# Graph-Machine-Learning-Group/sgp

Measured on AMD Instinct MI355X. Metric: encoded node-steps/sec, higher is better.
Workload: dtype f32 (hop products: operands as fp16 hi + lo pairs, three 16-bit MFMA terms per product, fp32 accumulation -- agrees with fp32 to ~1e-7 of the operand scale; reservoir: recurrent products: state (|h| <= 1, x 2^14) and W_hh (per-row power-of-two scale) as two fp16 pieces (22 bits), hi*hi + hi*lo + lo*

## Files before the change

include/sgp_amd.h:

```cpp
#ifndef SGP_AMD_H
#define SGP_AMD_H

#include <stdint.h>

#ifdef __cplusplus
extern "C" {
#endif

#define SGP_ABI_VERSION 4

#define SGP_EINVAL   (-1)
#define SGP_EUNSUP   (-2)
#define SGP_ENOMEM   (-3)

#define SGP_ACT_TANH      0
#define SGP_ACT_RELU      1
#define SGP_ACT_SELF_NORM 2
#define SGP_ACT_IDENTITY  3
#define SGP_ACT_TANH_REL  4

typedef void* sgp_stream_t;

int sgp_abi_version(void);
const char* sgp_last_error(void);
// ... 68 lines not shown
                       const float* x_tab, int32_t accumulate, int32_t t_chunk, const int32_t* pred, int32_t run_if, sgp_stream_t stream);
int32_t sgp_spmm_split_chunks(void);
int32_t sgp_spmm_split_max_union(void);
int32_t sgp_spmm_split_waves(void);
int32_t sgp_spmm_split_rows_per_wave(void);
int32_t sgp_spmm_split_max_feat(void);

int sgp_spmm_split_banded_f32(const int32_t* hdr, const int32_t* rowid, const int32_t* ucol, const void* afr,
                              const int32_t* adr, const float* rinv, int32_t n_tiles,
                              const float* X, int64_t x_row_stride, int64_t x_batch_stride,
                              const float* X_halo, int64_t xh_row_stride, int64_t xh_batch_stride, int32_t n_own,
                              float* Y, int64_t y_row_stride, int64_t y_batch_stride,
                              int32_t n_rows, int32_t n_cols, int32_t batch, int32_t feat,
                              const float* x_tab, int32_t accumulate, int32_t t_chunk,
                              int32_t walk, const int32_t* band_first, int32_t n_bands,
                              const int32_t* pred, int32_t run_if, sgp_stream_t stream);

int sgp_spmm_split_wide_f32(const int32_t* hdr, const int32_t* rowid, const int32_t* ucol, const void* afr,
                            const int32_t* adr, const float* rinv, int32_t n_tiles,
                            const float* X, int64_t x_row_stride, int64_t x_batch_stride,
                            const float* X_halo, int64_t xh_row_stride, int64_t xh_batch_stride, int32_t n_own,
                            float* Y, int64_t y_row_stride, int64_t y_batch_stride,
                            int32_t n_rows, int32_t n_cols, int32_t batch, int32_t feat,
                            const float* x_tab, int32_t accumulate, int32_t t_chunk, const int32_t* pred, int32_t run_if, sgp_stream_t stream);
int sgp_spmm_split_wide_banded_f32(const int32_t* hdr, const int32_t* rowid, const int32_t* ucol, const void* afr,
                                   const int32_t* adr, const float* rinv, int32_t n_tiles,
                                   const float* X, int64_t x_row_stride, int64_t x_batch_stride,
                                   const float* X_halo, int64_t xh_row_stride, int64_t xh_batch_stride, int32_t n_own,
                                   float* Y, int64_t y_row_stride, int64_t y_batch_stride,
                                   int32_t n_rows, int32_t n_cols, int32_t batch, int32_t feat,
                                   const float* x_tab, int32_t accumulate, int32_t t_chunk,
                                   int32_t walk, const int32_t* band_first, int32_t n_bands,
                                   const int32_t* pred, int32_t run_if, sgp_stream_t stream);
int32_t sgp_spmm_split_wide_chunks(void);
int32_t sgp_spmm_split_wide_max_union(void);
int32_t sgp_spmm_split_wide_waves(void);
int32_t sgp_spmm_split_wide_rows_per_wave(void);
int32_t sgp_spmm_split_wide_max_feat(void);

int sgp_split_plan_order(const int64_t* rowptr, const int64_t* col, int64_t nnz, int64_t n_rows, int64_t n_cols,
                         int32_t waves, int32_t chunks, int32_t max_union, int32_t rows_per_wave, int64_t* order);
int64_t sgp_split_plan_deal(const int64_t* rowptr, const int64_t* col, int64_t nnz, int64_t n_rows, int64_t n_cols,
                            const int64_t* order, int64_t n_order,
                            int32_t waves, int32_t chunks, int32_t max_union, int32_t rows_per_wave,
                            int64_t* wave_of_row, int64_t* slot_of_row, int64_t* tile_of_wave, int64_t* rows_of_wave);
int sgp_split_plan_fill(const int64_t* rowptr, const int64_t* col, const float* val, int64_t nnz, int64_t n_rows, int64_t n_cols,
                        const int64_t* wave_of_row, const int64_t* slot_of_row, const int64_t* tile_of_wave,
                        const int64_t* rows_of_wave, int64_t n_waves, int64_t n_tiles,
                        int32_t waves, int32_t chunks, int32_t max_union,
                        int32_t* hdr, int32_t* rowid, int32_t* ucol, void* afr, int32_t* adr, float* rinv,
                        double* stats, int32_t threads);
int64_t sgp_split_plan_bands(const int32_t* ucol, int64_t n_tiles, int32_t max_union, int64_t n_cols,
                             int64_t col_budget, int32_t* band_first);

int sgp_spmm_colblock_f32(const int32_t* plan, const int32_t* segptr, const int32_t* wg_row0,
                          int32_t n_wg, int32_t n_blocks,
                          const float* X, int64_t x_row_stride, int64_t x_batch_stride,
                          const float* X_halo, int64_t xh_row_stride, int64_t xh_batch_stride, int32_t n_own,
                          float* Y, int64_t y_row_stride, int64_t y_batch_stride,
                          int32_t n_rows, int32_t n_cols, int32_t batch, int32_t feat,
                          const int32_t* pred, int32_t run_if, sgp_stream_t stream);
int32_t sgp_spmm_colblock_rows_cap(void);
int32_t sgp_spmm_colblock_round_pad(void);

int32_t sgp_spmm_tiled_max_union(int32_t feat);
int32_t sgp_spmm_tiled_max_tile_rows(void);
int32_t sgp_spmm_tiled_max_row_edges(void);

int sgp_spmm_tiled_form(int32_t tile_rows, int32_t max_row_edges, int32_t* rows_per_group, int32_t* batches);
int32_t sgp_spmm_csr_form(int32_t feat, int32_t aligned, int32_t predicated);

int64_t sgp_reservoir_workspace_bytes(int32_t F, int32_t R);
int sgp_reservoir_f32(const float* x, int64_t x_row_stride, int64_t x_step_stride,
                      const float* w_ih, const float* w_hh, const float* b,
                      double alpha, int32_t act,
                      float* out, int64_t out_row_stride, int64_t out_step_stride,
                      float* h_state, void* workspace,
                      int32_t T, int32_t N, int32_t F, int32_t R,
                      sgp_stream_t stream);

int sgp_reservoir_pieces_f32(const float* x, int64_t x_row_stride, int64_t x_step_stride,
                             const float* w_ih, const float* w_hh, const float* b,
                             double alpha, int32_t act,
                             float* out, int64_t out_row_stride, int64_t out_step_stride,
                             float* h_state, void* workspace,
                             int32_t t_piece, int32_t t_last, int32_t n_pieces,
                             int64_t x_piece_stride, int64_t out_piece_stride, int32_t no_store,
                             int32_t N, int32_t F, int32_t R,
                             const int32_t* pred, int32_t run_if, sgp_stream_t stream);

int sgp_reservoir_describe(int32_t F, int32_t R, int32_t N, int32_t T, int32_t act, double alpha, int32_t has_state,
                           int32_t n_pieces, int32_t no_store, int32_t has_pred,
                           int64_t x_row_stride, int64_t x_step_stride, int32_t x_align,
                           int64_t out_row_stride, int64_t out_step_stride, int32_t out_align,
                           char* text, int64_t capacity);

int64_t sgp_reservoir_fused_workspace_bytes(int32_t F, int32_t R, int32_t L);
int32_t sgp_reservoir_fused_supported(int32_t F, int32_t R, int32_t L);
int sgp_reservoir_fused_f32(const float* x, int64_t x_row_stride, int64_t x_step_stride,
                            const float* const* w_ih, const float* const* w_hh, const float* const* b,
                            const double* alpha, int32_t act,
                            float* out, int64_t out_row_stride, int64_t out_step_stride,
                            float* h_state, void* workspace,
                            int32_t T, int32_t N, int32_t F, int32_t R, int32_t L,
                            sgp_stream_t stream);
int sgp_reservoir_fused_sums_f32(const float* x, int64_t x_row_stride, int64_t x_step_stride,
// ... 397 lines not shown
```

sgp_amd/csrc/plan_split.hip:

```cpp
#include "common.h"
#include <math.h>
#include <string.h>
#include <algorithm>
#include <atomic>
#include <new>
#include <system_error>
#include <thread>
#include <vector>

namespace {

constexpr int SET_SLOTS[4][8] = {{0, 1, 2, 3, 8, 9, 10, 11}, {4, 5, 6, 7, 12, 13, 14, 15},
                                 {16, 17, 18, 19, 24, 25, 26, 27}, {20, 21, 22, 23, 28, 29, 30, 31}};

inline uint16_t half_bits(_Float16 h) { uint16_t b; memcpy(&b, &h, 2); return b; }

inline void split_fp16(float v, uint16_t& hi, uint16_t& lo) {
    uint32_t bits;
    memcpy(&bits, &v, 4);
    bits &= 0xFFFFE000u;
    float hi32;
    memcpy(&hi32, &bits, 4);
    if (fabsf(v) < 6.103515625e-05f) hi32 = (float)(_Float16)v;
    const _Float16 h = (_Float16)hi32;
// ... 327 lines not shown
            w_mark[c] = wave;
            ++w_union;
            for (int64_t i = g.cp[c]; i < g.cp[c + 1]; ++i) {
                const int32_t q = g.cr[i];
                if (in_tile[q] != tile) continue;
                if (w_cnt_at[q] != wave) { w_cnt_at[q] = wave; w_cnt[q] = 0; }
                ++w_cnt[q];
            }
        }
    }
    int32_t cut_waves() {
        rest.assign(rows.begin(), rows.end());
        std::sort(rest.begin(), rest.end());
        for (int32_t r : rest) in_tile[r] = tile;
        wave_rows.clear();
        wave_first.assign(1, 0);
        while (!rest.empty()) {
            ++wave;
            w_union = 0;
            int32_t n_in = 0;
            size_t at = 0;
            for (;;) {
                const int32_t r = rest[at];
                rest.erase(rest.begin() + (int64_t)at);
                wave_take(r);
                if (++n_in == rows_per_wave || rest.empty()) break;
                at = 0;
                for (size_t i = 1; i < rest.size(); ++i) {
                    const int32_t q = rest[i], b = rest[at];
                    const int32_t nq = g.deg(q) - w_have(q), nb = g.deg(b) - w_have(b);
                    if (nq < nb || (nq == nb && w_have(q) > w_have(b))) at = i;
                }
                if (w_union + g.deg(rest[at]) - w_have(rest[at]) > wave_cols) break;
            }
            wave_first.push_back((int32_t)wave_rows.size());
        }
        return (int32_t)wave_first.size() - 1;
    }
    void run(int64_t* order) {
        int64_t n_out = 0;
        while (n_out < n_rows) {
            grow_tile();
            const int32_t n_waves = cut_waves();
            const int32_t kept = std::min(n_waves, waves);
            for (int32_t i = 0; i < wave_first[kept]; ++i) order[n_out++] = wave_rows[i];
            for (int32_t i = wave_first[kept]; i < wave_first[n_waves]; ++i) {
                placed[wave_rows[i]] = 0;
                next_row = std::min<int64_t>(next_row, wave_rows[i]);
            }
        }
    }
};

}

extern "C" int sgp_split_plan_order(const int64_t* rowptr, const int64_t* col, int64_t nnz, int64_t n_rows, int64_t n_cols,
                                    int32_t waves, int32_t chunks, int32_t max_union, int32_t rows_per_wave, int64_t* order) {
  return guarded<int>("sgp_split_plan_order", [&]() -> int {
    SGP_REQUIRE(rowptr && (col || nnz <= 0) && order, "sgp_split_plan_order: null pointer");
    SGP_REQUIRE(n_rows >= 0 && n_cols >= 0 && n_rows < (1ll << 31) - 1 && n_cols < (1ll << 31) - 1 && waves >= 1 && chunks >= 1 &&
                chunks <= (1 << 24) && max_union >= 1 && rows_per_wave >= 1 && (int64_t)waves * rows_per_wave < (1ll << 31),
                "sgp_split_plan_order: bad size");
    if (const char* f = rowptr_fault(rowptr, n_rows, nnz)) return sgp::fail(SGP_EINVAL, "sgp_split_plan_order: malformed CSR: %s", f);
    if (n_rows == 0) return 0;
    OrderGraph g;
    if (const char* f = order_graph(rowptr, col, n_rows, n_cols, g)) return sgp::fail(SGP_EINVAL, "sgp_split_plan_order: %s", f);
    Orderer(g, n_rows, n_cols, waves, chunks, max_union, rows_per_wave).run(order);
    return 0;
  });
}

extern "C" int sgp_split_plan_fill(const int64_t* rowptr, const int64_t* col, const float* val, int64_t nnz, int64_t n_rows, int64_t n_cols,
                                   const int64_t* wave_of_row, const int64_t* slot_of_row, const int64_t* tile_of_wave,
                                   const int64_t* rows_of_wave, int64_t n_waves, int64_t n_tiles,
                                   int32_t waves, int32_t chunks, int32_t max_union,
                                   int32_t* hdr, int32_t* rowid, int32_t* ucol, void* afr, int32_t* adr, float* rinv,
                                   double* stats, int32_t threads) {
  return guarded<int>("sgp_split_plan_fill", [&]() -> int {
    SGP_REQUIRE(rowptr && col && val && wave_of_row && slot_of_row && tile_of_wave && rows_of_wave && hdr && rowid && ucol &&
                afr && adr && rinv && stats, "sgp_split_plan_fill: null pointer");
    SGP_REQUIRE(n_rows > 0 && n_cols > 0 && n_waves > 0 && n_tiles > 0 && waves >= 1 && 2 * waves < 64 && chunks >= 1 &&
                max_union >= 1 && max_union <= 65536 / 64 * 8, "sgp_split_plan_fill: bad size");
    if (const char* f = rowptr_fault(rowptr, n_rows, nnz)) return sgp::fail(SGP_EINVAL, "sgp_split_plan_fill: malformed CSR: %s", f);
    for (int64_t e = 0; e < rowptr[n_rows]; ++e)
        SGP_REQUIRE(col[e] >= 0 && col[e] < n_cols, "sgp_split_plan_fill: column out of range");
    FillArgs a{rowptr, col, val, n_rows, n_cols, wave_of_row, slot_of_row, tile_of_wave, rows_of_wave, n_waves, n_tiles,
               waves, chunks, max_union, hdr, rowid, ucol, (uint16_t*)afr, adr, rinv};
    memset(hdr, 0, sizeof(int32_t) * 64 * n_tiles);
    std::fill(rowid, rowid + n_tiles * waves * 16, -1);
    std::fill(ucol, ucol + n_tiles * (int64_t)max_union, -1);
    memset(afr, 0, sizeof(uint16_t) * (size_t)n_tiles * waves * chunks * 2 * 512);
    memset(adr, 0, sizeof(int32_t) * (size_t)n_tiles * waves * chunks * 64);
    memset(rinv, 0, sizeof(float) * (size_t)n_tiles * waves * 16);
    std::vector<int64_t> first_wave(n_tiles + 1, 0), row_first(n_waves + 1, 0);
    for (int64_t w = 0; w < n_waves; ++w) {
        const int64_t t = tile_of_wave[w];
        SGP_REQUIRE(t >= 0 && t < n_tiles && (w == 0 || t == tile_of_wave[w - 1] || t == tile_of_wave[w - 1] + 1),
                    "sgp_split_plan_fill: tile_of_wave is not a non-decreasing run");
        SGP_REQUIRE(rows_of_wave[w] >= 0 && rows_of_wave[w] <= 16, "sgp_split_plan_fill: a wave holds at most 16 rows");
        ++first_wave[t + 1];
        row_first[w + 1] = row_first[w] + rows_of_wave[w];
    }
    for (int64_t t = 0; t < n_tiles; ++t) {
        SGP_REQUIRE(first_wave[t + 1] >= 1 && first_wave[t + 1] <= waves, "sgp_split_plan_fill: a tile holds 1 .. waves waves");
        first_wave[t + 1] += first_wave[t];
    }
// ... 90 lines not shown
```

sgp_amd/graph.py:

```python
from typing import NamedTuple

import numpy as np
import torch

from . import hip, tune
from .tileplan import build_reordered_plan, build_tile_plan, locality_order


def _as_edge_tensors(edge_index, edge_weight):
    if isinstance(edge_index, np.ndarray):
        edge_index = torch.from_numpy(edge_index)
        if edge_weight is not None and isinstance(edge_weight, np.ndarray):
            edge_weight = torch.from_numpy(edge_weight)
    if not torch.is_tensor(edge_index):
        raise RuntimeError("Edge index must be (edge_index, edge_weight) tuple "
                           "or SparseTensor.")
    ei = edge_index.detach().to("cpu", torch.long)
    ew = None if edge_weight is None else edge_weight.detach().to("cpu", torch.float32)
    return ei, ew


def _coalesce(row, col, val, n):
    key = row * n + col
    uniq, inv = torch.unique(key, sorted=True, return_inverse=True)
# ... 218 lines not shown
        key = ("colblock", feat, str(device))
        if key not in self._plans:
            plan = None
            from . import colblock
            if feat % 64 == 0 and self.num_cols < colblock.MAX_COLS and self.nnz() > 0:
                lib = hip.load()
                plan = colblock.build_colblock_plan(self.rowptr.numpy(), self.col.numpy(), self.val.numpy(),
                                                    self.num_nodes, self.num_cols, feat,
                                                    rows_cap=lib.sgp_spmm_colblock_rows_cap(),
                                                    round_pad=lib.sgp_spmm_colblock_round_pad(),
                                                    l2_bytes=tune.get("colblock_l2_mb", 2.5, float) * 2 ** 20)
                if plan is not None:
                    plan = plan.to(device)
            self._plans[key] = plan
        return self._plans[key]

    def mix_plan(self, feat, device, strict=True):
        key = ("mix", feat % 64 == 0, str(device), bool(strict))
        if key not in self._plans:
            plan = None
            base = self.tile_plan(feat, device, tall=False)
            if base is not None and base.pipe is not None and (base.group_fill >= 0.5 or not strict):
                from . import mixplan, plancache
                lib = hip.load()
                thr, dh = tune.get("mix_thr", 4, int), lib.sgp_spmm_mix_max_dense(int(self.num_cols > self.num_nodes))

                def build():
                    order = None
                    if base.reordered:
                        order = locality_order(self.rowptr.numpy(), self.col.numpy(), self.num_nodes)
                    return mixplan.build_mix_plan(self.rowptr.numpy(), self.col.numpy(), self.val.numpy(), self.num_nodes,
                                                  base, thr=thr, dh=dh, order=order)
                plan = plancache.fetch(self, "mix", (thr, dh, sorted(hip.tiled_limits(feat).items())), build)
                min_share = tune.get("mix_min_share", 0.25, float) if strict else -1.0
                if plan is not None and (plan.dense_share < min_share
                                         or plan.max_union > lib.sgp_spmm_mix_max_union()):
                    plan = None
                if plan is not None:
                    plan = plan.to(device)
            self._plans[key] = plan
        return self._plans[key]

    def split_plan(self, device):
        key = ("split", str(device))
        if key not in self._plans:
            plan = None
            if self.nnz() > 0:
                from . import plancache
                lib = hip.load()
                lim, wide = hip.split_limits(), hip.split_limits(wide=True)
                if tune.get("split_wide", 1, int) == 0:
                    wide = None
                plan = plancache.fetch(self, "split", (sorted(lim.items()), wide and sorted(wide.items()),
                                                       tune.get("split_passes", 1, int), _split_order_mode()),
                                       lambda: self._build_split_plan(lim, wide))
                if isinstance(plan, list):
                    plan = SplitPasses(p.to(device) for p in plan)
                elif plan is not None:
                    plan = plan.to(device)
            self._plans[key] = plan
        return self._plans[key]

    def _build_split_plan(self, lim, wide=None):
        from . import splitplan
        args = (self.rowptr.numpy(), self.col.numpy(), self.val.numpy(), self.num_nodes, self.num_cols)
        bands = dict(band_cols=SPLIT_BAND_BYTES // 256)
        plan = splitplan.build_split_plan(*args, **lim, **bands)
        if plan is not None and plan.stats["rows_per_wave"] < 0.75 * lim["rows_per_wave"] and self.num_nodes >= 2048 and \
                self.num_cols == self.num_nodes:
            alt = splitplan.build_split_plan(*args, order=locality_order(
                self.rowptr.numpy(), self.col.numpy(), self.num_nodes), **lim, **bands)
            if alt is not None and alt.stats["staged_per_row"] < plan.stats["staged_per_row"]:
                plan = alt
                plan.stats["order"] = "locality"
        mode = _split_order_mode()
        if plan is not None and mode != "off" and self.num_cols == self.num_nodes:
            given = plan.stats["tiles"]
            blob = splitplan.blob_order(*args[:2], *args[3:], **lim)
            tiles = splitplan.deal_tiles(*args[:2], *args[3:], order=blob, **lim)
            if tiles is not None and (tiles < given or mode == "on"):
                plan = splitplan.build_split_plan(*args, order=blob, **lim, **bands)
                plan.stats["order"] = "blob"
            plan.stats.setdefault("order", "numbering")
            plan.stats.update(split_order=mode, tiles_given=given, tiles_blob=tiles)
        if plan is not None and (plan.stats["rows_per_wave"] < 0.375 * lim["rows_per_wave"] or
                                 plan.stats["staged_per_row"] > 8):
            plan = None
        if plan is None and self.max_degree() > 32 * lim["chunks"] and tune.get("split_passes", 1, int) != 0:
            deg = (self.rowptr[1:] - self.rowptr[:-1])
            if wide is not None and float((deg > 32 * lim["chunks"]).float().mean()) < 0.5:
                wide = None
            passes = splitplan.build_split_passes(*args, max_passes=12, **(wide or lim), **bands)
            if passes is not None and passes[0].stats["rows_per_wave"] >= 0.5 * lim["rows_per_wave"] and \
                    passes[0].stats["staged_per_row"] <= 8:
                plan = list(passes)
            elif wide is not None:
                return self._build_split_plan(lim, None)
        return plan

    def prepare(self, feat, device, halo=False):
        self.device_csr(device)
        if self.nnz() == 0:
            return ["csr"]
        c = self._select(feat, device, _NOMINAL)
        made = (["split"] if c.split is not None else []) + (["tile"] if c.tile is not None else [])
        if c.lazy:
            return made + ["csr (behind the split hop's predicate until a flag asks for the exact kernels)"]
        made += {"spmm_mix": ["mix"], "spmm_colblock": ["colblock"]}.get(c.kernel, [])
        return made or ["csr"]

    def split_eligible(self, x, y, halo=None):
        return self._select(x.shape[2], x.device, _operands(x, y, halo, None), split_only=True).split is not None

    def norm_inf(self):
        if not hasattr(self, "_norm_inf"):
            rp = self.rowptr.long()
            sums = torch.zeros(self.num_nodes, dtype=torch.float64)
            if self.nnz():
                sums.index_add_(0, torch.repeat_interleave(torch.arange(self.num_nodes), rp[1:] - rp[:-1]),
                                self.val.double().abs())
            self._norm_inf = float(sums.max()) if self.num_nodes else 0.0
        return self._norm_inf

    def propagate(self, x, y, force=None, halo=None, x_bound=None):
        if (halo is None) != (self.num_cols == self.num_nodes):
            raise ValueError("halo rows are required exactly when num_cols > num_nodes")
        if x.dim() != 3 or y.dim() != 3 or y.shape[0] != x.shape[0] or y.shape[2] != x.shape[2]:
            raise ValueError("propagate expects [B, N, F] operands of equal batch and feature size")
        n_src = x.shape[1] + (0 if halo is None else halo.shape[1])
        if n_src != self.num_cols or y.shape[1] != self.num_nodes:
            raise ValueError(f"operand shapes do not match the operator: {n_src} source rows for "
                             f"{self.num_cols} columns, {y.shape[1]} result rows for {self.num_nodes}")
        if halo is not None and (halo.shape[0] != x.shape[0] or halo.shape[2] != x.shape[2]):
            raise ValueError("halo batch / feature size differs from x")
        if force not in (None, "csr", "tiled", "res", "mix", "colblock", "split"):
            raise ValueError(f"unknown kernel {force!r} (csr, tiled, res, mix, colblock, split)")
        if x.shape[0] == 0 or x.shape[2] == 0 or self.num_nodes == 0:
# ... 118 lines not shown
        if not self._flag_pending:
            return
        still = []
        for slot, ev in self._flag_pending:
            if ev.query():
                if int(self._flag_host[slot]) == 0:
                    self._exact_seen = True
            else:
                still.append((slot, ev))
        self._flag_pending = still

    def index_select(self, dim, index):
        if dim != 0:
            raise NotImplementedError("only row selection (dim=0) is used by the reference")
        idx = torch.as_tensor(index, dtype=torch.long).cpu()
        rp = self.rowptr.long()
        counts = (rp[1:] - rp[:-1])[idx]
        new_rp = torch.zeros(idx.numel() + 1, dtype=torch.long)
        new_rp[1:] = torch.cumsum(counts, 0)
        take = torch.repeat_interleave(rp[idx] - new_rp[:-1], counts) + torch.arange(int(new_rp[-1]))
        return ShiftOperator(new_rp, self.col[take], self.val[take], idx.numel(), num_cols=self.num_cols)

    def propagate_rect(self, x, y):
        if x.shape[1] != self.num_cols or y.shape[1] != self.num_nodes:
            raise ValueError("operand shapes do not match the operator")
        if self.num_cols == self.num_nodes:
            return self.propagate(x, y)
        rowptr, col, val = self.device_csr(x.device)
        hip.spmm_csr(rowptr, col, val, x, y)
        return y

    def __matmul__(self, x):
        if not torch.is_tensor(x) or x.dim() < 2:
            raise TypeError("ShiftOperator @ expects a dense tensor [..., N, F]")
        lead = x.shape[:-2]
        x3 = x.reshape(-1, x.shape[-2], x.shape[-1])
        if x3.dtype != torch.float32:
            x3 = x3.float()
        if x3.stride(2) != 1:
            x3 = x3.contiguous()
        if x3.shape[1] != self.num_cols:
            raise ValueError(f"operand has {x3.shape[1]} rows, the operator {self.num_cols} columns")
        on_cpu = not x3.is_cuda
        if on_cpu:
            hip.require_gpu()
            x3 = x3.cuda()
        y = torch.empty(x3.shape[0], self.num_nodes, x3.shape[2], dtype=torch.float32, device=x3.device)
        self.propagate_rect(x3, y)
        if on_cpu:
            y = y.cpu()
        return y.reshape(*lead, self.num_nodes, x.shape[-1])


def _split_order_mode():
    mode = tune.get("split_order", "auto")
    if mode not in ("off", "on", "auto"):
        raise ValueError(f"SGP_TUNE: split_order={mode!r} is not one of off, on, auto")
    return mode


class SplitPasses(list):

    @property
    def stats(self):
        return self[0].stats

    @property
    def n_tiles(self):
        return sum(p.n_tiles for p in self)
```

sgp_amd/plancache.py:

```python
import hashlib
import os
import tempfile

import torch

VERSION = 9
_dir = None
stats = {"hits": 0, "misses": 0, "stores": 0}


def set_dir(path):
    global _dir
    _dir = path


def directory():
    return _dir or os.environ.get("SGP_AMD_CACHE") or None


def operator_hash(op):
    h = getattr(op, "_csr_hash", None)
    if h is None:
        m = hashlib.blake2b(digest_size=16)
        m.update(f"{op.num_nodes}:{op.num_cols}:{op.nnz()}".encode())
        for t in (op.rowptr, op.col, op.val):
            m.update(t.contiguous().numpy().tobytes())
        h = op._csr_hash = m.hexdigest()
    return h


def _path(op, kind, params):
    d = directory()
    if d is None:
        return None
    tag = hashlib.blake2b(repr((VERSION, kind, params)).encode(), digest_size=8).hexdigest()
    return os.path.join(d, f"{kind}-{operator_hash(op)}-{tag}.pt")


_MISS = object()


def fetch(op, kind, params, build):
    path = _path(op, kind, params)
    if path is None:
        return build()
    if os.path.exists(path):
        try:
            got = torch.load(path, map_location="cpu", weights_only=False)
            if isinstance(got, dict) and got.get("version") == VERSION and got.get("params") == repr(params):
                stats["hits"] += 1
                return got["plan"]
        except Exception:
            pass
    stats["misses"] += 1
    plan = build()
    try:
        os.makedirs(os.path.dirname(path), exist_ok=True)
        fd, tmp = tempfile.mkstemp(dir=os.path.dirname(path), suffix=".tmp")
        os.close(fd)
# ... 7 lines not shown
```

sgp_amd/splitplan.py:

```python
import numpy as np
import torch


class SplitPlan:
    def __init__(self, hdr, rowid, ucol, afr, adr, rinv, n_tiles, n_rows, n_cols, norm_inf, stats):
        self.hdr, self.rowid, self.ucol, self.afr, self.adr, self.rinv = hdr, rowid, ucol, afr, adr, rinv
        self.n_tiles, self.n_rows, self.n_cols = n_tiles, n_rows, n_cols
        self.norm_inf, self.stats = norm_inf, stats
        self.accumulate = False
        self.bands = {}
        self.ucol_host = ucol if ucol.device.type == "cpu" else None

    def __setstate__(self, state):
        self.__dict__.update(state)
        self.__dict__.setdefault("bands", {})
        self.__dict__.setdefault("ucol_host", self.ucol if self.ucol.device.type == "cpu" else None)

    def to(self, device):
        p = SplitPlan(self.hdr.to(device), self.rowid.to(device), self.ucol.to(device), self.afr.to(device),
                      self.adr.to(device), self.rinv.to(device), self.n_tiles, self.n_rows, self.n_cols, self.norm_inf,
                      self.stats)
        p.accumulate = self.accumulate
        p.bands = {k: (t.to(device), m) for k, (t, m) in self.bands.items()}
        p.ucol_host = self.ucol_host
        return p

    def band_table(self, col_budget):
        col_budget = int(col_budget)
        if col_budget not in self.bands:
            host = self.ucol_host if self.ucol_host is not None else self.ucol.cpu()
            first = build_bands(host, self.n_cols, col_budget)
            self.bands[col_budget] = (first.to(self.ucol.device), int((first[1:] - first[:-1]).max()))
        return self.bands[col_budget]

    def describe(self):
        st = self.stats
        line = (f"split plan: {st['tiles']} tiles, {st['rows_per_tile']:.1f} rows per tile, {st['rows_per_wave']:.2f} rows per wave, "
                f"{st['staged_per_row']:.2f} staged rows per result row")
        if "order" in st:
            line += (f"; rows dealt in {st['order']} order (SGP_TUNE split_order={st['split_order']}: "
                     f"{st['tiles_given']} tiles in the given order, {st['tiles_blob']} in blob order)")
        return line


def build_bands(ucol, n_cols, col_budget):
    from . import hip
    lib = hip.load()
    ucol = ucol.contiguous()
    assert ucol.dtype == torch.int32 and ucol.dim() == 2 and ucol.device.type == "cpu"
    n_tiles = ucol.shape[0]
    first = torch.empty(n_tiles + 1, dtype=torch.int32)
    n = lib.sgp_split_plan_bands(ucol.data_ptr(), n_tiles, ucol.shape[1], int(n_cols), int(col_budget), first.data_ptr())
    if n < 0:
        raise (MemoryError if n == -3 else RuntimeError)("sgp_split_plan_bands: " + lib.sgp_last_error().decode())
    return first[:n + 1].clone()


def _host_csr(rowptr, col, n_rows):
    rowptr = np.ascontiguousarray(rowptr, dtype=np.int64)
    col = np.ascontiguousarray(col, dtype=np.int64)
    if rowptr.size < n_rows + 1:
        raise ValueError("rowptr is shorter than n_rows + 1")
    return rowptr, col


def blob_order(rowptr, col, n_rows, n_cols, waves=16, chunks=7, max_union=768, rows_per_wave=16):
    import ctypes
    from . import hip
    lib = hip.load()
    rowptr, col = _host_csr(rowptr, col, n_rows)
    ptr = lambda a: a.ctypes.data_as(ctypes.c_void_p)
    order = np.empty(n_rows, dtype=np.int64)
    rc = lib.sgp_split_plan_order(ptr(rowptr), ptr(col), col.size, n_rows, n_cols, waves, chunks, max_union, rows_per_wave, ptr(order))
    if rc != 0:
        raise (MemoryError if rc == -3 else ValueError)("sgp_split_plan_order: " + lib.sgp_last_error().decode())
    return order


def deal_tiles(rowptr, col, n_rows, n_cols, waves=16, chunks=7, max_union=768, rows_per_wave=16, order=None):
    import ctypes
    from . import hip
    lib = hip.load()
    rowptr, col = _host_csr(rowptr, col, n_rows)
    seq = None if order is None else np.ascontiguousarray(order, dtype=np.int64)
    ptr = lambda a: a.ctypes.data_as(ctypes.c_void_p)
    out = [np.empty(max(n_rows, 1), dtype=np.int64) for _ in range(4)]
    n_waves = lib.sgp_split_plan_deal(ptr(rowptr), ptr(col), col.size, n_rows, n_cols, None if seq is None else ptr(seq),
                                      0 if seq is None else seq.size, waves, chunks, max_union, rows_per_wave, *map(ptr, out))
    if n_waves == -2 or n_waves == 0:
        return None
    if n_waves < 0:
        raise (MemoryError if n_waves == -3 else RuntimeError)("sgp_split_plan_deal: " + lib.sgp_last_error().decode())
    return int(out[2][n_waves - 1]) + 1


def deal_rows(rowptr, col, n_rows, n_cols, waves, chunks, max_union, rows_per_wave=32, order=None):
    cap = 32 * chunks
    wmark = np.full(n_cols, -1, dtype=np.int64)
    tmark = np.full(n_cols, -1, dtype=np.int64)
    wave_of_row = np.full(n_rows, -1, dtype=np.int64)
    slot_of_row = np.full(n_rows, -1, dtype=np.int64)
    tile_of_wave, rows = [], []
    wave, tile = -1, -1
    w_rows = w_cols = t_cols = t_waves = 0

    def open_wave(r, new_tile):
        nonlocal wave, tile, w_rows, w_cols, t_cols, t_waves
        wave += 1
        if new_tile:
            tile += 1
            t_cols = t_waves = 0
        t_waves += 1
        w_rows = w_cols = 0
        tile_of_wave.append(tile)
        rows.append(0)

    for r in (range(n_rows) if order is None else order):
        r = int(r)
        c = np.unique(col[rowptr[r]:rowptr[r + 1]])
        if c.size > cap or c.size > max_union:
            return None
        if wave < 0:
            open_wave(r, True)
        new_w = int((wmark[c] != wave).sum())
        new_t = int((tmark[c] != tile).sum())
        need_wave = w_rows == rows_per_wave or w_cols + new_w > cap
        if t_cols + new_t > max_union or (need_wave and t_waves == waves):
            open_wave(r, True)
            new_w = new_t = c.size
        elif need_wave:
            open_wave(r, False)
            new_w = c.size
        wmark[c] = wave
        tmark[c] = tile
        w_cols += new_w
        t_cols += new_t
        wave_of_row[r] = wave
        slot_of_row[r] = w_rows
        w_rows += 1
        rows[wave] = w_rows
    return (wave_of_row, slot_of_row, np.asarray(tile_of_wave, dtype=np.int64), np.asarray(rows, dtype=np.int64))


def split_fp16(v):
    v = np.asarray(v, dtype=np.float32)
    bits = v.view(np.uint32) & np.uint32(0xFFFFE000)
    hi32 = bits.view(np.float32)
    small = np.abs(v) < np.float32(2.0 ** -14)
    hi32 = np.where(small, v.astype(np.float16).astype(np.float32), hi32)
    hi = hi32.astype(np.float16)
    lo = (v - hi.astype(np.float32)).astype(np.float16)
    return hi, lo


_SET_SLOTS = np.array([[0, 1, 2, 3, 8, 9, 10, 11], [4, 5, 6, 7, 12, 13, 14, 15],
                       [16, 17, 18, 19, 24, 25, 26, 27], [20, 21, 22, 23, 28, 29, 30, 31]])


def _bank_aware_slots(w_of_key, pos_of_key, stage, n_chunks_total, chunks):
    chunk = pos_of_key // 32
    wc = w_of_key * chunks + chunk
    res = stage & 7
    idx = np.arange(wc.size)

    def rank_within(group, *minor):
        order = np.lexsort(tuple(reversed(minor)) + (group,))
        g = group[order]
        first = np.r_[True, g[1:] != g[:-1]]
        start = np.maximum.accumulate(np.where(first, idx, 0))
        out = np.empty_like(idx)
        out[order] = idx - start
        return out

    rank = rank_within(wc * 8 + res, stage)
    primary = rank < 4
    slot = np.full(wc.size, -1, dtype=np.int64)
    j = rank_within(np.where(primary, wc * 4 + rank, -1), res)
    slot[primary] = _SET_SLOTS[rank[primary], j[primary]]
    occ = np.zeros((n_chunks_total, 32), dtype=bool)
    occ[wc[primary], slot[primary]] = True
    extra = ~primary
    if extra.any():
        free = np.argsort(occ, axis=1, kind="stable")
        e = rank_within(np.where(extra, wc, -1), res, stage)
        slot[extra] = free[wc[extra], e[extra]]
    return chunk * 32 + slot


def build_split_plan(rowptr, col, val, n_rows, n_cols, waves=16, chunks=7, max_union=768, order=None, rows_per_wave=16,
                     threads=0, band_cols=None):
    import ctypes
    from . import hip
    lib = hip.load()
    rowptr = np.ascontiguousarray(rowptr, dtype=np.int64)
    col = np.ascontiguousarray(col, dtype=np.int64)
    val = np.ascontiguousarray(val, dtype=np.float32)
    if n_rows == 0 or col.size == 0 or not np.isfinite(val).all():
        return None
    assert rows_per_wave == 16 and rowptr.size >= n_rows + 1 and val.size == col.size
    if col.min() < 0 or col.max() >= n_cols:
        raise ValueError("column index out of range")
    seq = None if order is None else np.ascontiguousarray(order, dtype=np.int64)
    ptr = lambda a: a.ctypes.data_as(ctypes.c_void_p)
    wave_of_row, slot_of_row = np.empty(n_rows, dtype=np.int64), np.empty(n_rows, dtype=np.int64)
    tile_of_wave, rows = np.empty(n_rows, dtype=np.int64), np.empty(n_rows, dtype=np.int64)
    n_waves = lib.sgp_split_plan_deal(ptr(rowptr), ptr(col), col.size, n_rows, n_cols, None if seq is None else ptr(seq),
                                      0 if seq is None else seq.size, waves, chunks, max_union, rows_per_wave,
                                      ptr(wave_of_row), ptr(slot_of_row), ptr(tile_of_wave), ptr(rows))
    if n_waves == -2 or n_waves == 0:
        return None
    if n_waves < 0:
        raise (MemoryError if n_waves == -3 else RuntimeError)("sgp_split_plan_deal: " + lib.sgp_last_error().decode())
    tile_of_wave, rows = tile_of_wave[:n_waves], rows[:n_waves]
    n_tiles = int(tile_of_wave[-1]) + 1
    hdr = torch.empty((n_tiles, 64), dtype=torch.int32)
    rowid = torch.empty((n_tiles, waves, rows_per_wave), dtype=torch.int32)
    ucol = torch.empty((n_tiles, max_union), dtype=torch.int32)
    afr = torch.empty((n_tiles, waves, chunks, 2, 64, 8), dtype=torch.float16)
    adr = torch.empty((n_tiles, waves, chunks, 64), dtype=torch.int32)
    rinv = torch.empty((n_tiles, waves, 16), dtype=torch.float32)
    st = np.zeros(8, dtype=np.float64)
    hip._check(lib.sgp_split_plan_fill(ptr(rowptr), ptr(col), ptr(val), col.size, n_rows, n_cols, ptr(wave_of_row), ptr(slot_of_row),
                                       ptr(tile_of_wave), ptr(rows), n_waves, n_tiles, waves, chunks, max_union,
                                       hdr.data_ptr(), rowid.data_ptr(), ucol.data_ptr(), afr.data_ptr(), adr.data_ptr(),
                                       rinv.data_ptr(), ptr(st), int(threads)), "sgp_split_plan_fill")
    stats = dict(tiles=n_tiles, waves=int(n_waves), rows_per_wave=float(st[2]), rows_per_tile=float(st[3]),
                 staged_per_row=float(st[4]), chunk_fill=float(st[5]), max_union=int(st[6]))
    plan = SplitPlan(hdr, rowid, ucol, afr, adr, rinv, n_tiles, n_rows, n_cols, float(st[7]), stats)
    if band_cols:
        plan.band_table(band_cols)
    return plan


def build_split_plan_numpy(rowptr, col, val, n_rows, n_cols, waves=16, chunks=7, max_union=768, order=None, rows_per_wave=16):
    rowptr = np.asarray(rowptr, dtype=np.int64)
    col = np.asarray(col, dtype=np.int64)
    val = np.asarray(val, dtype=np.float32)
    if n_rows == 0 or col.size == 0 or not np.isfinite(val).all():
        return None
    assert rows_per_wave == 16
    deal = deal_rows(rowptr, col, n_rows, n_cols, waves, chunks, max_union, rows_per_wave=rows_per_wave, order=order)
    if deal is None:
        return None
    wave_of_row, slot_of_row, tile_of_wave, rows = deal
    n_waves = tile_of_wave.size
    n_tiles = int(tile_of_wave[-1]) + 1
    first_wave_of_tile = np.searchsorted(tile_of_wave, np.arange(n_tiles))
    w_in_tile = np.arange(n_waves) - first_wave_of_tile[tile_of_wave]

    row_of_edge = np.repeat(np.arange(n_rows, dtype=np.int64), np.diff(rowptr[:n_rows + 1]))
    rowsum = np.zeros(n_rows, dtype=np.float64)
    np.add.at(rowsum, row_of_edge, np.abs(val.astype(np.float64)))
    dealt = wave_of_row[row_of_edge] >= 0
    row_of_edge, col, val = row_of_edge[dealt], col[dealt], val[dealt]
    e_wave = wave_of_row[row_of_edge]
    e_tile = tile_of_wave[e_wave]
    tkey, tinv = np.unique(e_tile * n_cols + col, return_inverse=True)
    t_of_key = tkey // n_cols
    t_first = np.searchsorted(t_of_key, np.arange(n_tiles))
    union = np.diff(np.append(t_first, tkey.size))
    stage_of_key = np.arange(tkey.size) - t_first[t_of_key]
    ucol = np.full((n_tiles, max_union), -1, dtype=np.int32)
    ucol[t_of_key, stage_of_key] = (tkey % n_cols).astype(np.int32)
    empty = union == 0
    ucol[empty, 0] = 0
# ... 131 lines not shown
```

Measured before the change: 1.339 billion.

## Refill under-full split-plan tiles by dissolving neighbouring tiles into them

Adds a host-side refill pass after the split-plan deal. It tries to dissolve small neighbouring tiles, greedily placing their rows into under-full tiles within the union-column and wave limits, with a repair step when the recut needs too many waves. In auto mode the refilled plan is used only when it produces fewer tiles. Fewer, fuller tiles are meant to cut per-tile staging overhead and workgroup count in the SpMM, at the cost of extra plan-build time and possibly larger per-tile column unions.

```diff
diff --git a/include/sgp_amd.h b/include/sgp_amd.h
--- a/include/sgp_amd.h
+++ b/include/sgp_amd.h
@@ -144,6 +144,10 @@
                         double* stats, int32_t threads);
 int64_t sgp_split_plan_bands(const int32_t* ucol, int64_t n_tiles, int32_t max_union, int64_t n_cols,
                              int64_t col_budget, int32_t* band_first);
+int64_t sgp_split_plan_refill(const int64_t* rowptr, const int64_t* col, int64_t nnz, int64_t n_rows, int64_t n_cols,
+                              int32_t waves, int32_t chunks, int32_t max_union, int32_t rows_per_wave,
+                              int64_t* wave_of_row, int64_t* slot_of_row, int64_t* tile_of_wave, int64_t* rows_of_wave,
+                              int64_t n_waves, int64_t* info);
 
 int sgp_spmm_colblock_f32(const int32_t* plan, const int32_t* segptr, const int32_t* wg_row0,
                           int32_t n_wg, int32_t n_blocks,
diff --git a/sgp_amd/csrc/plan_split.hip b/sgp_amd/csrc/plan_split.hip
--- a/sgp_amd/csrc/plan_split.hip
+++ b/sgp_amd/csrc/plan_split.hip
@@ -403,6 +403,272 @@
     }
 };
 
+struct Refiller {
+    using Waves = std::vector<std::vector<int32_t>>;
+    const OrderGraph& g;
+    Orderer cut;
+    const int64_t n_rows;
+    const int32_t waves, wave_cols, max_union, rows_per_wave;
+    const size_t cap_rows;
+    std::vector<Waves> t_waves;
+    std::vector<int32_t> t_size, tile_of_row;
+    std::vector<int32_t> c_mark, c_loc, c_loc_at, r_have, r_pool, t_seen;
+    std::vector<int64_t> failed_at;
+    std::vector<int32_t> nb, nb_d, recv, pool, taken, cand;
+    std::vector<std::pair<int32_t, Waves>> journal;
+    std::vector<uint8_t> cnt;
+    std::vector<int32_t> wc;
+    int32_t stamp = 0, n_loc = 0;
+    int64_t commits = 0, repaired = 0;
+
+    Refiller(const OrderGraph& g_, int64_t n_rows_, int64_t n_cols, int32_t waves_, int32_t chunks, int32_t max_union_, int32_t rpw)
+        : g(g_), cut(g_, n_rows_, n_cols, waves_, chunks, max_union_, rpw), n_rows(n_rows_), waves(waves_), wave_cols(32 * chunks),
+          max_union(max_union_), rows_per_wave(rpw), cap_rows((size_t)waves_ * rpw), tile_of_row(n_rows_, -1),
+          c_mark(n_cols, 0), c_loc(n_cols, 0), c_loc_at(n_cols, 0), r_have(n_rows_, 0), r_pool(n_rows_, 0) {}
+
+    const char* load(const int64_t* wave_of_row, const int64_t* slot_of_row, const int64_t* tile_of_wave, const int64_t* rows_of_wave,
+                     int64_t n_waves) {
+        if (tile_of_wave[0] != 0) return "tile_of_wave does not start at 0";
+        for (int64_t w = 0; w < n_waves; ++w) {
+            if (w && tile_of_wave[w] != tile_of_wave[w - 1] && tile_of_wave[w] != tile_of_wave[w - 1] + 1) return "tile_of_wave is not a non-decreasing run";
+            if (rows_of_wave[w] < 1 || rows_of_wave[w] > rows_per_wave) return "a wave holds 1 .. rows_per_wave rows";
+        }
+        int64_t n_slots = 0;
+        for (int64_t w = 0; w < n_waves; ++w) n_slots += rows_of_wave[w];
+        if (n_slots != n_rows) return "rows_of_wave does not add up to the rows";
+        const int64_t n_tiles = tile_of_wave[n_waves - 1] + 1;
+        t_waves.assign((size_t)n_tiles, Waves());
+        for (int64_t w = 0; w < n_waves; ++w) t_waves[tile_of_wave[w]].emplace_back((size_t)rows_of_wave[w], -1);
+        std::vector<int64_t> first_wave((size_t)n_tiles, 0);
+        for (int64_t w = n_waves - 1; w >= 0; --w) first_wave[tile_of_wave[w]] = w;
+        for (int64_t r = 0; r < n_rows; ++r) {
+            const int64_t w = wave_of_row[r];
+            if (w < 0 || w >= n_waves) return "a row without a wave (the refill takes deals of every row)";
+            const int64_t t = tile_of_wave[w];
+            std::vector<int32_t>& wv = t_waves[t][w - first_wave[t]];
+            if (slot_of_row[r] < 0 || slot_of_row[r] >= (int64_t)wv.size() || wv[slot_of_row[r]] >= 0) return "wave / slot of a row inconsistent";
+            wv[slot_of_row[r]] = (int32_t)r;
+            tile_of_row[r] = (int32_t)t;
+        }
+        t_size.assign((size_t)n_tiles, 0);
+        for (int64_t t = 0; t < n_tiles; ++t) {
+            if ((int64_t)t_waves[t].size() > waves) return "a tile holds at most `waves` waves";
+            for (const auto& wv : t_waves[t]) t_size[t] += (int32_t)wv.size();
+        }
+        t_seen.assign((size_t)n_tiles, 0);
+        failed_at.assign((size_t)n_tiles, -1);
+        return nullptr;
+    }
+    void neighbours(int32_t x, std::vector<int32_t>& out) {
+        const int32_t s = ++stamp;
+        out.clear();
+        for (const auto& wv : t_waves[x])
+            for (int32_t r : wv)
+                for (int64_t e = g.rp[r]; e < g.rp[r + 1]; ++e) {
+                    const int32_t c = g.rc[e];
+                    if (c_mark[c] == s) continue;
+                    c_mark[c] = s;
+                    for (int64_t i = g.cp[c]; i < g.cp[c + 1]; ++i) {
+                        const int32_t t = tile_of_row[g.cr[i]];
+                        if (t != x && t_seen[t] != s) { t_seen[t] = s; out.push_back(t); }
+                    }
+                }
+    }
+    void cut_into(const std::vector<int32_t>& rows, Waves& wv) {
+        ++cut.tile;
+        cut.rows = rows;
+        const int32_t n = cut.cut_waves();
+        wv.assign((size_t)n, std::vector<int32_t>());
+        for (int32_t w = 0; w < n; ++w) wv[w].assign(cut.wave_rows.begin() + cut.wave_first[w], cut.wave_rows.begin() + cut.wave_first[w + 1]);
+    }
+    uint8_t& at(size_t w, int32_t c) { return cnt[w * (size_t)n_loc + c_loc[c]]; }
+    int32_t fresh(size_t w, int32_t r) {
+        int32_t n = 0;
+        for (int64_t e = g.rp[r]; e < g.rp[r + 1]; ++e) n += at(w, g.rc[e]) == 0;
+        return n;
+    }
+    void add(size_t w, int32_t r) { for (int64_t e = g.rp[r]; e < g.rp[r + 1]; ++e) wc[w] += at(w, g.rc[e])++ == 0; }
+    void sub(size_t w, int32_t r) { for (int64_t e = g.rp[r]; e < g.rp[r + 1]; ++e) wc[w] -= --at(w, g.rc[e]) == 0; }
+    bool repair(Waves& wv) {
+        while ((int32_t)wv.size() > waves) {
+            const size_t n_w = wv.size();
+            size_t s = 0;
+            for (size_t w = 1; w < n_w; ++w) if (wv[w].size() <= wv[s].size()) s = w;
+            const int32_t st = ++stamp;
+            n_loc = 0;
+            for (const auto& rows : wv)
+                for (int32_t r : rows)
+                    for (int64_t e = g.rp[r]; e < g.rp[r + 1]; ++e)
+                        if (c_loc_at[g.rc[e]] != st) { c_loc_at[g.rc[e]] = st; c_loc[g.rc[e]] = n_loc++; }
+            cnt.assign(n_w * (size_t)std::max(n_loc, 1), 0);
+            wc.assign(n_w, 0);
+            for (size_t w = 0; w < n_w; ++w) for (int32_t r : wv[w]) add(w, r);
+            const Waves before(wv);
+            const std::vector<int32_t> leaving(wv[s]);
+            for (int32_t y : leaving) {
+                size_t to = n_w;
+                int32_t to_new = 0;
+                for (size_t a = 0; a < n_w; ++a) {
+                    if (a == s || (int32_t)wv[a].size() >= rows_per_wave) continue;
+                    const int32_t nw = fresh(a, y);
+                    if (wc[a] + nw <= wave_cols && (to == n_w || nw < to_new)) { to = a; to_new = nw; }
+                }
+                if (to < n_w) { add(to, y); wv[to].push_back(y); continue; }
+                bool done = false;
+                for (size_t a = 0; a < n_w && !done; ++a) {
+                    if (a == s) continue;
+                    for (size_t xi = 0; xi < wv[a].size() && !done; ++xi) {
+                        const int32_t x = wv[a][xi];
+                        sub(a, x);
+                        if (wc[a] + fresh(a, y) <= wave_cols)
+                            for (size_t b = 0; b < n_w && !done; ++b) {
+                                if (b == s || b == a || (int32_t)wv[b].size() >= rows_per_wave || wc[b] + fresh(b, x) > wave_cols) continue;
+                                add(a, y); wv[a][xi] = y;
+                                add(b, x); wv[b].push_back(x);
+                                done = true;
+                            }
+                        if (!done) add(a, x);
+                    }
+                }
+                if (!done) { wv = before; return false; }
+            }
+            wv.erase(wv.begin() + (int64_t)s);
+            ++repaired;
+        }
+        return true;
+    }
+    void place(int32_t t) {
+        const int32_t s = ++stamp;
+        int32_t u = 0;
+        for (const auto& wv : t_waves[t])
+            for (int32_t r : wv)
+                for (int64_t e = g.rp[r]; e < g.rp[r + 1]; ++e)
+                    if (c_mark[g.rc[e]] != s) { c_mark[g.rc[e]] = s; ++u; }
+        for (int32_t q : pool) {
+            r_pool[q] = s;
+            r_have[q] = 0;
+            for (int64_t e = g.rp[q]; e < g.rp[q + 1]; ++e) r_have[q] += c_mark[g.rc[e]] == s;
+        }
+        taken.clear();
+        const size_t room = cap_rows - (size_t)t_size[t];
+        while (taken.size() < room) {
+            int32_t best = -1;
+            for (int32_t q : pool) {
+                if (r_pool[q] != s) continue;
+                if (best < 0) { best = q; continue; }
+                const int32_t nq = g.deg(q) - r_have[q], nb_ = g.deg(best) - r_have[best];
+                if (nq < nb_ || (nq == nb_ && r_have[q] > r_have[best])) best = q;
+            }
+            if (best < 0 || u + g.deg(best) - r_have[best] > max_union) break;
+            r_pool[best] = 0;
+            taken.push_back(best);
+            for (int64_t e = g.rp[best]; e < g.rp[best + 1]; ++e) {
+                const int32_t c = g.rc[e];
+                if (c_mark[c] == s) continue;
+                c_mark[c] = s;
+                ++u;
+                for (int64_t i = g.cp[c]; i < g.cp[c + 1]; ++i) if (r_pool[g.cr[i]] == s) ++r_have[g.cr[i]];
+            }
+        }
+        Waves wv;
+        size_t m = taken.size();
+        while (m > 0) {
+            cand.clear();
+            for (const auto& w : t_waves[t]) cand.insert(cand.end(), w.begin(), w.end());
+            cand.insert(cand.end(), taken.begin(), taken.begin() + (int64_t)m);
+            cut_into(cand, wv);
+            if ((int32_t)wv.size() <= waves || repair(wv)) break;
+            size_t over = 0;
+            for (size_t w = (size_t)waves; w < wv.size(); ++w) over += wv[w].size();
+            m -= std::min(m, std::max<size_t>(1, over));
+        }
+        if (m == 0) return;
+        journal.emplace_back(t, std::move(wv));
+        for (size_t i = 0; i < m; ++i) r_pool[taken[i]] = -1;
+        pool.erase(std::remove_if(pool.begin(), pool.end(), [&](int32_t q) { return r_pool[q] == -1; }), pool.end());
+    }
+    bool try_dissolve(int32_t d, int32_t first) {
+        neighbours(d, nb_d);
+        std::sort(nb_d.begin(), nb_d.end());
+        recv.assign(1, first);
+        size_t slack = cap_rows - (size_t)t_size[first];
+        for (int32_t t : nb_d)
+            if (t != first && (size_t)t_size[t] < cap_rows) { recv.push_back(t); slack += cap_rows - (size_t)t_size[t]; }
+        if (slack < (size_t)t_size[d]) return false;
+        pool.clear();
+        for (const auto& wv : t_waves[d]) pool.insert(pool.end(), wv.begin(), wv.end());
+        std::sort(pool.begin(), pool.end());
+        journal.clear();
+        for (size_t i = 0; i < recv.size() && !pool.empty(); ++i) place(recv[i]);
+        if (!pool.empty()) return false;
+        for (auto& j : journal) {
+            t_waves[j.first] = std::move(j.second);
+            t_size[j.first] = 0;
+            for (const auto& wv : t_waves[j.first]) {
+                t_size[j.first] += (int32_t)wv.size();
+                for (int32_t r : wv) tile_of_row[r] = j.first;
+            }
+        }
+        t_waves[d].clear();
+        t_size[d] = 0;
+        return true;
+    }
+    void run() {
+        const int32_t n_tiles = (int32_t)t_waves.size();
+        for (int32_t t = 0; t < n_tiles; ++t) {
+            bool moved = true;
+            while (moved && t_size[t] > 0 && (size_t)t_size[t] < cap_rows) {
+                moved = false;
+                neighbours(t, nb);
+                std::sort(nb.begin(), nb.end(), [&](int32_t a, int32_t b) { return t_size[a] != t_size[b] ? t_size[a] < t_size[b] : a < b; });
+                for (int32_t d : nb) {
+                    if ((size_t)t_size[d] >= cap_rows) break;
+                    if (failed_at[d] == commits) continue;
+                    if (try_dissolve(d, t)) { ++commits; moved = true; break; }
+                    failed_at[d] = commits;
+                }
+            }
+        }
+    }
+    int64_t store(int64_t* wave_of_row, int64_t* slot_of_row, int64_t* tile_of_wave, int64_t* rows_of_wave) const {
+        int64_t wave = 0, tile = 0;
+        for (const Waves& tw : t_waves) {
+            if (tw.empty()) continue;
+            for (const auto& wv : tw) {
+                for (size_t i = 0; i < wv.size(); ++i) { wave_of_row[wv[i]] = wave; slot_of_row[wv[i]] = (int64_t)i; }
+                tile_of_wave[wave] = tile;
+                rows_of_wave[wave++] = (int64_t)wv.size();
+            }
+            ++tile;
+        }
+        return wave;
+    }
+};
+
+}
+
+extern "C" int64_t sgp_split_plan_refill(const int64_t* rowptr, const int64_t* col, int64_t nnz, int64_t n_rows, int64_t n_cols,
+                                         int32_t waves, int32_t chunks, int32_t max_union, int32_t rows_per_wave,
+                                         int64_t* wave_of_row, int64_t* slot_of_row, int64_t* tile_of_wave, int64_t* rows_of_wave,
+                                         int64_t n_waves, int64_t* info) {
+  return guarded<int64_t>("sgp_split_plan_refill", [&]() -> int64_t {
+    SGP_REQUIRE(rowptr && (col || nnz <= 0) && wave_of_row && slot_of_row && tile_of_wave && rows_of_wave && info,
+                "sgp_split_plan_refill: null pointer");
+    SGP_REQUIRE(n_rows >= 1 && n_cols >= 1 && n_rows < (1ll << 31) - 1 && n_cols < (1ll << 31) - 1 && waves >= 1 && chunks >= 1 &&
+                chunks <= (1 << 24) && max_union >= 1 && rows_per_wave >= 1 && rows_per_wave <= 255 &&
+                (int64_t)waves * rows_per_wave < (1ll << 31) && n_waves >= 1 && n_waves <= n_rows, "sgp_split_plan_refill: bad size");
+    if (const char* f = rowptr_fault(rowptr, n_rows, nnz)) return sgp::fail(SGP_EINVAL, "sgp_split_plan_refill: malformed CSR: %s", f);
+    OrderGraph g;
+    if (const char* f = order_graph(rowptr, col, n_rows, n_cols, g)) return sgp::fail(SGP_EINVAL, "sgp_split_plan_refill: %s", f);
+    Refiller refill(g, n_rows, n_cols, waves, chunks, max_union, rows_per_wave);
+    if (const char* f = refill.load(wave_of_row, slot_of_row, tile_of_wave, rows_of_wave, n_waves))
+        return sgp::fail(SGP_EINVAL, "sgp_split_plan_refill: %s", f);
+    info[0] = (int64_t)refill.t_waves.size();
+    refill.run();
+    info[1] = info[0] - refill.commits;
+    info[2] = refill.repaired;
+    return refill.store(wave_of_row, slot_of_row, tile_of_wave, rows_of_wave);
+  });
 }
 
 extern "C" int sgp_split_plan_order(const int64_t* rowptr, const int64_t* col, int64_t nnz, int64_t n_rows, int64_t n_cols,
diff --git a/sgp_amd/graph.py b/sgp_amd/graph.py
--- a/sgp_amd/graph.py
+++ b/sgp_amd/graph.py
@@ -294,7 +294,8 @@
                 if tune.get("split_wide", 1, int) == 0:
                     wide = None
                 plan = plancache.fetch(self, "split", (sorted(lim.items()), wide and sorted(wide.items()),
-                                                       tune.get("split_passes", 1, int), _split_order_mode()),
+                                                       tune.get("split_passes", 1, int), _split_order_mode(),
+                                                       _split_refill_mode()),
                                        lambda: self._build_split_plan(lim, wide))
                 if isinstance(plan, list):
                     plan = SplitPasses(p.to(device) for p in plan)
@@ -307,13 +308,13 @@
         from . import splitplan
         args = (self.rowptr.numpy(), self.col.numpy(), self.val.numpy(), self.num_nodes, self.num_cols)
         bands = dict(band_cols=SPLIT_BAND_BYTES // 256)
-        plan = splitplan.build_split_plan(*args, **lim, **bands)
+        plan, order = splitplan.build_split_plan(*args, **lim, **bands), None
         if plan is not None and plan.stats["rows_per_wave"] < 0.75 * lim["rows_per_wave"] and self.num_nodes >= 2048 and \
                 self.num_cols == self.num_nodes:
-            alt = splitplan.build_split_plan(*args, order=locality_order(
-                self.rowptr.numpy(), self.col.numpy(), self.num_nodes), **lim, **bands)
+            local = locality_order(self.rowptr.numpy(), self.col.numpy(), self.num_nodes)
+            alt = splitplan.build_split_plan(*args, order=local, **lim, **bands)
             if alt is not None and alt.stats["staged_per_row"] < plan.stats["staged_per_row"]:
-                plan = alt
+                plan, order = alt, local
                 plan.stats["order"] = "locality"
         mode = _split_order_mode()
         if plan is not None and mode != "off" and self.num_cols == self.num_nodes:
@@ -321,10 +322,18 @@
             blob = splitplan.blob_order(*args[:2], *args[3:], **lim)
             tiles = splitplan.deal_tiles(*args[:2], *args[3:], order=blob, **lim)
             if tiles is not None and (tiles < given or mode == "on"):
-                plan = splitplan.build_split_plan(*args, order=blob, **lim, **bands)
+                plan, order = splitplan.build_split_plan(*args, order=blob, **lim, **bands), blob
                 plan.stats["order"] = "blob"
             plan.stats.setdefault("order", "numbering")
             plan.stats.update(split_order=mode, tiles_given=given, tiles_blob=tiles)
+        refill = _split_refill_mode()
+        if plan is not None and refill != "off" and self.num_cols == self.num_nodes:
+            dealt, stats = plan.stats["tiles"], plan.stats
+            tiles = splitplan.deal_tiles(*args[:2], *args[3:], order=order, refill=True, **lim)
+            if tiles < dealt or refill == "on":
+                plan = splitplan.build_split_plan(*args, order=order, refill=True, **lim, **bands)
+                plan.stats.update({k: stats[k] for k in ("order", "split_order", "tiles_given", "tiles_blob") if k in stats})
+            plan.stats.update(split_refill=refill, tiles_dealt=dealt, tiles_refill=tiles, refilled=tiles < dealt or refill == "on")
         if plan is not None and (plan.stats["rows_per_wave"] < 0.375 * lim["rows_per_wave"] or
                                  plan.stats["staged_per_row"] > 8):
             plan = None
@@ -549,6 +558,13 @@
         return y.reshape(*lead, self.num_nodes, x.shape[-1])
 
 
+def _split_refill_mode():
+    mode = tune.get("split_refill", "auto")
+    if mode not in ("off", "on", "auto"):
+        raise ValueError(f"SGP_TUNE: split_refill={mode!r} is not one of off, on, auto")
+    return mode
+
+
 def _split_order_mode():
     mode = tune.get("split_order", "auto")
     if mode not in ("off", "on", "auto"):
diff --git a/sgp_amd/plancache.py b/sgp_amd/plancache.py
--- a/sgp_amd/plancache.py
+++ b/sgp_amd/plancache.py
@@ -4,7 +4,7 @@
 
 import torch
 
-VERSION = 9
+VERSION = 10
 _dir = None
 stats = {"hits": 0, "misses": 0, "stores": 0}
 
diff --git a/sgp_amd/splitplan.py b/sgp_amd/splitplan.py
--- a/sgp_amd/splitplan.py
+++ b/sgp_amd/splitplan.py
@@ -40,6 +40,9 @@
         if "order" in st:
             line += (f"; rows dealt in {st['order']} order (SGP_TUNE split_order={st['split_order']}: "
                      f"{st['tiles_given']} tiles in the given order, {st['tiles_blob']} in blob order)")
+        if "split_refill" in st:
+            line += (f"; under-full tiles {'refilled' if st['refilled'] else 'left as dealt'} (SGP_TUNE split_refill={st['split_refill']}: "
+                     f"{st['tiles_dealt']} tiles as dealt, {st['tiles_refill']} refilled)")
         return line
 
 
@@ -77,7 +80,15 @@
     return order
 
 
-def deal_tiles(rowptr, col, n_rows, n_cols, waves=16, chunks=7, max_union=768, rows_per_wave=16, order=None):
+def _refill(lib, ptr, rowptr, col, n_rows, n_cols, lim, deal, n_waves):
+    info = np.zeros(3, dtype=np.int64)
+    n = lib.sgp_split_plan_refill(ptr(rowptr), ptr(col), col.size, n_rows, n_cols, *lim, *map(ptr, deal), n_waves, ptr(info))
+    if n <= 0:
+        raise (MemoryError if n == -3 else ValueError)("sgp_split_plan_refill: " + lib.sgp_last_error().decode())
+    return int(n)
+
+
+def deal_tiles(rowptr, col, n_rows, n_cols, waves=16, chunks=7, max_union=768, rows_per_wave=16, order=None, refill=False):
     import ctypes
     from . import hip
     lib = hip.load()
@@ -91,6 +102,8 @@
         return None
     if n_waves < 0:
         raise (MemoryError if n_waves == -3 else RuntimeError)("sgp_split_plan_deal: " + lib.sgp_last_error().decode())
+    if refill:
+        n_waves = _refill(lib, ptr, rowptr, col, n_rows, n_cols, (waves, chunks, max_union, rows_per_wave), out, n_waves)
     return int(out[2][n_waves - 1]) + 1
 
 
@@ -188,7 +201,7 @@
 
 
 def build_split_plan(rowptr, col, val, n_rows, n_cols, waves=16, chunks=7, max_union=768, order=None, rows_per_wave=16,
-                     threads=0, band_cols=None):
+                     threads=0, band_cols=None, refill=False):
     import ctypes
     from . import hip
     lib = hip.load()
@@ -211,6 +224,9 @@
         return None
     if n_waves < 0:
         raise (MemoryError if n_waves == -3 else RuntimeError)("sgp_split_plan_deal: " + lib.sgp_last_error().decode())
+    if refill:
+        n_waves = _refill(lib, ptr, rowptr, col, n_rows, n_cols, (waves, chunks, max_union, rows_per_wave),
+                          (wave_of_row, slot_of_row, tile_of_wave, rows), n_waves)
     tile_of_wave, rows = tile_of_wave[:n_waves], rows[:n_waves]
     n_tiles = int(tile_of_wave[-1]) + 1
     hdr = torch.empty((n_tiles, 64), dtype=torch.int32)
```

After: 1.328 billion. About the same (-0.8%).
